# HAHHHD/mllp

Measured on AMD Instinct MI355X. Metric: LP instances/sec (fwd+bwd) on Netlib batch; achieved HBM GB/s on CSR SpMM, higher is better.
Workload: dtype f32; 1 GPU; netlib_full: BASELINE.json configs[2], 97 instances / 1,074,147 nnz per global batch, one block-diagonal batch per GPU, one Adam step per global batch: fwd + BCE + bwd + gradient all-reduce + Adam, fp32; global_batch=97, instances_rank0=97, nnz_rank0=1074147, hip_graph=False, parallelism=dp1

## Files before the change

### mllp_amd/csrc/api.cpp

```cpp
#include <algorithm>

#include "internal.h"

namespace mllp {

static inline int64_t up16(int64_t x) { return (x + 15) & ~int64_t(15); }

ConvWs conv_ws_carve(float* base, int64_t n, int cin, float** end) {
    const int64_t recw = cin == 16 ? REC_W : 8;
    float* p = base;
    auto take = [&](int64_t floats) {
        float* q = p;
        p += up16(floats);
        return q;
    };
    ConvWs w;
    w.derived = take(DERIVED_W);
    w.qp = take(n * cin);
    w.t = take(n);
    w.Z = take(n * cin);
    w.aux = take(n * 4);
    w.rec = take(n * recw);
    w.dqp = take(n * cin);
    w.dsdt = take(n * 2);
// ... 154 lines not shown
    TRY(c1v.pre(s));
    TRY(c1v.dst(s));
    TRY(c1v.stat(s));
    TRY(c1c.pre(a));
    TRY(c1c.dst(a));
    TRY(c1c.stat(a));
#undef REC
#undef WAIT
    TRY(fork_to(a, s, g->ev[0]));
#undef TRY
    return model_finalize(g, P, w, false, grads, s);
}

static bool use_fused(const mllp_graph* g) {
    if (g->path == 1 || !g->fused_built) return false;
    if (g->path == 2) return true;
    return g->nnz < ((int64_t)32 << 20);
}

}

using namespace mllp;

extern "C" int mllp_spmm_csr_f32(const mllp_graph_t* g, int transpose, const float* d_H, float* d_Y, void* stream) {
    REQUIRE(g && d_H && d_Y, "null argument");
    const Orient& o = transpose ? g->At : g->A;
    return launch_spmm(o, d_H, d_Y, o.scratch, (hipStream_t)stream);
}

extern "C" int mllp_spmm_csr_bf16(const mllp_graph_t* g, int transpose, const void* d_H_bf16, float* d_Y, void* stream) {
    REQUIRE(g && d_H_bf16 && d_Y, "null argument");
    const Orient& o = transpose ? g->At : g->A;
    const Tiled& tl = o.tiled[TILED_SPMM];
// ... 2 lines not shown
    if (tl.n_tiles == 0) {
        if (o.n_dst > 0) MLLP_HIP_TRY(hipMemsetAsync(d_Y, 0, (size_t)o.n_dst * 16 * sizeof(float), (hipStream_t)stream));
        return MLLP_OK;
    }
    return launch_spmm_tiled_bf16(tl, o.n_dst, o.n_src, d_H_bf16, d_Y, (hipStream_t)stream);
}

extern "C" int mllp_graph_invalidate_inputs(mllp_graph_t* g) {
    REQUIRE(g, "null graph");
    g->bound_x1 = g->bound_x2 = g->bound_labels = nullptr;
    return MLLP_OK;
}

extern "C" int mllp_graph_set_path(mllp_graph_t* g, int path) {
    REQUIRE(g, "null graph");
    REQUIRE(path >= 0 && path <= 2, "path must be 0 (by size), 1 (generic / LDS-tiled sweeps) or 2 (fused latency-regime kernels)");
    if (path == 2 && !g->fused_built) {
        const int rc = fused_graph_build(g, g->h_csr_ptr.data(), g->h_csc_ptr.data());
        if (rc) return rc;
    }
    g->path = path;
    g->folded_ws = g->folded_params = nullptr;
    return MLLP_OK;
}

extern "C" int mllp_tiled_geometry(int variant, int32_t* rows_per_tile, int32_t* cols_per_block,
                                   int32_t* bundle_capacity) {
    REQUIRE(rows_per_tile && cols_per_block && bundle_capacity, "null argument");
    REQUIRE(variant >= 0 && variant <= 4, "variant must be 0 (SpMM), 1 (attention forward), 2 / 4 (attention backward, source- / destination-major) or 3 (layer-1 sweeps)");
    int a, b, c;
    tiled_geometry(variant, &a, &b, &c);
    *rows_per_tile = a; *cols_per_block = b; *bundle_capacity = c;
// ... 117 lines not shown
                       d_logits, nullptr, w.head_partials, s);
}

extern "C" int mllp_gnn_backward(const mllp_graph_t* g, const float* d_params, const float* d_x1, const float* d_x2,
                                 void* d_ws, const float* d_dlogits, float* d_grads, void* stream) {
    REQUIRE(g && d_params && d_x1 && d_x2 && d_ws && d_dlogits && d_grads, "null argument");
    hipStream_t s = (hipStream_t)stream;
    ModelWs w = model_ws(g, (float*)d_ws);
    int rc;
    REQUIRE(g->ws_ptr == d_ws && g->ws_path == (use_fused(g) ? 1 : 0),
            "no mllp_gnn_forward on this workspace with the current path (mllp_graph_set_path between forward and backward?)");
    if (use_fused(g)) {
        const FusedModel m{d_params, w, d_x1, d_x2, nullptr, 0.0f, nullptr};
        if ((rc = fused_bind(const_cast<mllp_graph*>(g), d_x1, d_x2, nullptr, s))) return rc;
        if ((rc = fused_head_backward(g, m, d_dlogits, s))) return rc;
        return fused_backward(g, m, false, d_grads, nullptr, s);
    }
    if ((rc = launch_head(1, g->N, w.h3v, d_params + OFF_FC, d_params + OFF_FC + FEAT, g->inv_n, nullptr, 0.0f,
                          d_dlogits, nullptr, w.d3v, w.head_partials, s))) return rc;
    if ((rc = fork_to(s, g->aux, g->ev[1]))) return rc;
    if ((rc = launch_head_finalize(w.head_partials, head_blocks_for(g->N), d_grads + OFF_FC, nullptr, g->aux))) return rc;
    return model_backward_body(g, d_params, d_x1, d_x2, w, d_grads, s);
}

static int input_grads_body(const mllp_graph* g, const float* x1, const float* x2, const ModelWs& w, float* dx1,
                            float* dx2, float* dval, hipStream_t s) {
    int rc;
    auto edge = [&](int c, const float* x_src, int accumulate) {
        const bool t = MODEL_CONV[c].dst_is_var;
        return launch_edge_grad(t ? g->At : g->A, g->nnz, MODEL_CONV[c].cin, w.c[c], x_src, t ? g->at_pos : nullptr, dval,
                                accumulate, s);
// ... 5 lines not shown
    if ((rc = edge(CONV_1C, x1, 0)) || (rc = edge(CONV_2C, w.h1v, 1)) || (rc = edge(CONV_1V, x2, 1)) ||
        (rc = edge(CONV_2V, w.h1c, 1))) return rc;
    return edge(CONV_3V, w.h2c, 1);
}

extern "C" int mllp_gnn_loss_step(const mllp_graph_t* g, const float* d_params, const float* d_x1, const float* d_x2,
                                  const float* d_labels, float inv_batch, void* d_ws, float* d_logits, float* d_loss,
                                  float* d_grads, void* stream) {
    REQUIRE(g && d_params && d_x1 && d_x2 && d_labels && d_ws && d_logits && d_loss && d_grads, "null argument");
    hipStream_t s = (hipStream_t)stream;
    ModelWs w = model_ws(g, (float*)d_ws);
    int rc;
    const_cast<mllp_graph*>(g)->folded_ws = const_cast<mllp_graph*>(g)->folded_params = nullptr;
    if (use_fused(g)) {
        const FusedModel m{d_params, w, d_x1, d_x2, d_labels, inv_batch, d_logits};
        if ((rc = fused_forward(const_cast<mllp_graph*>(g), m, 2, s))) return rc;
        return fused_backward(g, m, true, d_grads, d_loss, s);
    }
    if ((rc = model_forward_body(g, d_params, d_x1, d_x2, w, s))) return rc;
    if ((rc = launch_head(2, g->N, w.h3v, d_params + OFF_FC, d_params + OFF_FC + FEAT, g->inv_n, d_labels, inv_batch,
                          nullptr, d_logits, w.d3v, w.head_partials, s))) return rc;
    if ((rc = fork_to(s, g->aux, g->ev[1]))) return rc;
    if ((rc = launch_head_finalize(w.head_partials, head_blocks_for(g->N), d_grads + OFF_FC, d_loss, g->aux))) return rc;
    return model_backward_body(g, d_params, d_x1, d_x2, w, d_grads, s);
}

extern "C" int mllp_gnn_input_grads_scratch_bytes(const mllp_graph_t* g, int64_t* bytes) {
    REQUIRE(g && bytes, "null argument");
    *bytes = up16(MLLP_NUM_PARAMS) * (int64_t)sizeof(float);
    return MLLP_OK;
}

// ... 18 lines not shown
extern "C" int mllp_gnn_train_step(const mllp_graph_t* g, float* d_params, const float* d_x1, const float* d_x2,
                                   const float* d_labels, float inv_batch, void* d_ws, float* d_logits, float* d_loss,
                                   float* d_grads, float* d_exp_avg, float* d_exp_avg_sq, float* d_state, float eps,
                                   int flags, void* stream) {
    REQUIRE(g && d_params && d_x1 && d_x2 && d_labels && d_ws && d_logits && d_loss && d_grads, "null argument");
    REQUIRE(d_exp_avg && d_exp_avg_sq && d_state, "null optimizer state");
    REQUIRE((flags & ~1) == 0, "flags: bit 0 = the folded weights in the workspace are current");
    hipStream_t s = (hipStream_t)stream;
    int rc;
    mllp_graph* gm = const_cast<mllp_graph*>(g);
    if (use_fused(g)) {
        ModelWs w = model_ws(g, (float*)d_ws);
        const FusedModel m{d_params, w, d_x1, d_x2, d_labels, inv_batch, d_logits};
        const bool skip = (flags & 1) != 0 && gm->folded_ws == d_ws && gm->folded_params == d_params;
        gm->folded_ws = gm->folded_params = nullptr;
        if ((rc = fused_forward(gm, m, 2, s, skip))) return rc;
        const FusedAdam a = {d_params, d_exp_avg, d_exp_avg_sq, d_state, eps, (int)MLLP_NUM_PARAMS};
        if ((rc = fused_backward(g, m, true, d_grads, d_loss, s, &a))) return rc;
        gm->folded_ws = d_ws;
        gm->folded_params = d_params;
        return MLLP_OK;
    }
    gm->folded_ws = gm->folded_params = nullptr;
    if ((rc = mllp_gnn_loss_step(g, d_params, d_x1, d_x2, d_labels, inv_batch, d_ws, d_logits, d_loss, d_grads, stream)))
        return rc;
    return launch_adam(d_params, d_grads, d_exp_avg, d_exp_avg_sq, d_state, eps, 1.0f, MLLP_NUM_PARAMS, s);
}

extern "C" int mllp_gnn_small_step_limits(int64_t limits[4]) {
    REQUIRE(limits, "null argument");
    limits[0] = SMALL_STEP_MAX_NODES; limits[1] = SMALL_STEP_MAX_NNZ;
    limits[2] = SMALL_STEP_THREADS; limits[3] = SMALL_STEP_LDS_BYTES;
    return MLLP_OK;
// ... 70 lines not shown
```

### mllp_amd/csrc/fused_kernels.hip

```cpp
#include <algorithm>
#include <vector>

#include "device_utils.h"
#include "host_graph.h"
#include "internal.h"
#include "node_bodies.h"

namespace mllp {

typedef float f32x4m __attribute__((ext_vector_type(4)));

#ifdef MLLP_TIMING_BUILD
static int g_fused_abl = [] {
    const char* e = getenv("MLLP_FUSED_ABL");
    return e ? atoi(e) : 0;
}();
#define FUSED_ABL(bit) ((J.abl & (bit)) != 0)
__device__ unsigned long long g_fused_stamps[8192 * 8];
__device__ unsigned long long g_fused_stamps1[8192 * 8];
#define FUSED_STAMP(k)                                                                      \
    {                                                                                       \
        __builtin_amdgcn_sched_barrier(0);                                                  \
        const unsigned long long now_ = __builtin_amdgcn_s_memtime();                       \
        __builtin_amdgcn_sched_barrier(0);                                                  \
        stamp_sum[k] += now_ - stamp_last;                                                  \
        stamp_last = now_;                                                                  \
    }
#else
#define FUSED_ABL(bit) false
#define FUSED_STAMP(k)
#endif

constexpr int FT = 768;
constexpr int FW = FT / 64;
constexpr int RT = 1024;
constexpr int MAXJOBS = 2;

constexpr int NP = FUSED_NP;
static_assert(NP == FUSED_PARTS, "partition count");

struct PartTiers {
    int row0, n_block, n_wave, n_group, n_base;
};
struct ItemsDev {
    const int* __restrict__ sptr;
// ... 321 lines not shown
        if (J.head == 2) *reinterpret_cast<float4*>(J.g_out + (size_t)p.row * 16 + 4 * part) = p.g;
    }
    p.row = -1;
}

struct FwdNext {
    RowSlot r;
    float4 xd;
    int2 en;
    int lrow;
    SlotReq q;
};
__device__ __forceinline__ void fwd16_row(const FwdJob16& J, const FwdW16& W, const PartTiers& P, const RowSlot& r,
                                          const float4& xd, int2& en, int lrow, const SlotReq& q1, int it2, FwdNext& nx,
                                          FwdPending& pend, int part, int lane, float* merge_lds, float* tiles, HeadAcc& ha
#ifdef MLLP_TIMING_BUILD
                                          , unsigned long long (&stamp_sum)[8], unsigned long long& stamp_last
#endif
) {
    FUSED_STAMP(0)
    const int n_mine = FUSED_ABL(256) ? 0 : slot_count(r);
    Gather4 gt;
    gather4_issue(J.s, J.x_src, r, n_mine, 0, part, en, gt);
    nx.r = slot_make(q1);
    nx.xd = ld4(J.x_dst + (size_t)max(nx.r.row, 0) * 16 + 4 * part);
    nx.en = first_entries_any<4>(J.s, nx.r, part);
    nx.lrow = J.perm[max(nx.r.row, 0)];
    nx.q = item_request<4>(J.s, P, max(it2, 0), lane);
    float4 qp;
    float t;
    {
        float ax_[4];
        tile_put(tiles, xd, lane);
        tile_rows(tiles, lane, ax_);
// ... 95 lines not shown
    ha.b = wave_sum(ha.b);
    ha.l = wave_sum(ha.l);
    if (lane < 4) {
        float* d = head_lds + wave * 18 + 4 * lane;
        d[0] = ha.w.x; d[1] = ha.w.y; d[2] = ha.w.z; d[3] = ha.w.w;
    }
    if (lane == 0) { head_lds[wave * 18 + 16] = ha.b; head_lds[wave * 18 + 17] = ha.l; }
    __syncthreads();
    if (tid < 18) {
        float v = 0.0f;
        for (int w = 0; w < NW; ++w) v += head_lds[w * 18 + tid];
        head_part[(size_t)blockIdx.x * 18 + tid] = v;
    }
}

__global__ __launch_bounds__(FT) void fused_fwd16_kernel(FwdLaunch16 A) {
    __shared__ FwdW16 Ws_[MAXJOBS];
    __shared__ float merge_lds[FW * 20];
    __shared__ float head_lds[FW * 18];
    __shared__ float tiles_[FW * 3 * TILE];
    const int tid = threadIdx.x, lane = tid & 63, wave = tid >> 6, part = lane & 3;
    for (int j = 0; j < A.n_jobs; ++j) {
        const FwdJob16& J = A.job[j];
        FwdW16& W = Ws_[j];
        if (wave == 0) matB_store(W.BPq, matB(J.D + OFF_PQ, 16, lane), lane);
        if (wave == 1) matB_store(W.BWv, matB(J.p.Wv, 16, lane), lane);
        if (wave == 2) matB_store(W.BWs, matB(J.p.Ws, 16, lane), lane);
        if (tid < 16) {
            W.pq0[tid] = J.D[OFF_PQ0 + tid];
            W.Pt[tid] = J.D[OFF_PT + tid];
            W.bv[tid] = J.p.bv[tid];
            W.we[tid] = J.p.we[tid];
            W.bs[tid] = J.p.bs[tid];
            W.fcw[tid] = J.head ? J.fcw[tid] : 0.0f;
        }
        if (tid == 0) {
            W.pt0 = J.D[OFF_PT0];
            W.fcb = J.head ? J.fcb[0] : 0.0f;
        }
    }
    __syncthreads();
    float* tiles = tiles_ + wave * 3 * TILE;
    HeadAcc ha;
    ha.w = f4zero(); ha.b = 0.0f; ha.l = 0.0f;
#ifdef MLLP_TIMING_BUILD
    unsigned long long stamp_sum[8] = {0, 0, 0, 0, 0, 0, 0, 0};
    unsigned long long stamp_last = __builtin_amdgcn_s_memtime();
    const unsigned long long stamp_begin = stamp_last;
#define STAMP_ARGS , stamp_sum, stamp_last
#else
#define STAMP_ARGS
#endif
    const int px = blockIdx.x % NP, bi = blockIdx.x / NP, gp = gridDim.x / NP;
    const int gw = bi * FW + wave;
    float* head_part = nullptr;
    for (int j = 0; j < A.n_jobs; ++j) {
        const FwdJob16& J = A.job[j];
        const PartTiers P = J.s.part[px];
        if (J.head == 2) head_part = J.head_part;
        const RowSlot none = empty_slot();
        FwdPending pend;
        pend.row = -1;
        for (int k = bi; k < P.n_block; k += gp) {
            const RowSlot r = block_slot<4>(J.s, P.row0 + k, tid);
            const float4 xd = ld4(J.x_dst + (size_t)r.row * 16 + 4 * part);
            int2 en = first_entries<4>(J.s, r, part);
            const int lrow = J.head ? J.perm[r.row] : 0;
            FwdNext nx;
            fwd16_row(J, Ws_[j], P, r, xd, en, lrow, empty_request(), -1, nx, pend, part, lane, merge_lds, tiles, ha STAMP_ARGS);
        }
        WaveList wl = wave_list(J.s, px, gw);
        for (int c0 = 0; c0 < wl.L; c0 += 64) {
            wave_list_chunk(wl, c0, lane);
            int it = wave_list_get(wl, 0), it1 = wave_list_get(wl, 1);
            RowSlot r = it >= 0 ? item_slot<4>(J.s, P, it, lane) : none;
            float4 xd = r.row >= 0 ? ld4(J.x_dst + (size_t)r.row * 16 + 4 * part) : f4zero();
            int2 en = first_entries<4>(J.s, r, part);
            int lrow = (J.head && r.row >= 0) ? J.perm[r.row] : 0;
            SlotReq q1 = item_request<4>(J.s, P, max(it1, 0), lane);
            if (it1 < 0) q1.row = -1;
            asm volatile("" : "+v"(xd.x), "+v"(xd.y), "+v"(xd.z), "+v"(xd.w), "+v"(en.x), "+v"(en.y), "+v"(lrow),
                              "+v"(q1.sb), "+v"(q1.se));
            for (int k = 0; it >= 0; ++k) {
                const int it2 = wave_list_get(wl, k + 2);
                FwdNext nx;
                fwd16_row(J, Ws_[j], P, r, xd, en, lrow, q1, it2, nx, pend, part, lane, merge_lds, tiles, ha STAMP_ARGS);
#ifdef MLLP_TIMING_BUILD
                stamp_sum[7] += 1;
#endif
                r = nx.r; xd = nx.xd; en = nx.en; lrow = nx.lrow; q1 = nx.q;
                it = it1; it1 = it2;
            }
        }
        fwd16_flush(J, pend, part);
    }
#ifdef MLLP_TIMING_BUILD
    if (lane == 0 && A.job[0].abl >= 0) {
        stamp_sum[6] = __builtin_amdgcn_s_memtime() - stamp_begin;
        unsigned long long* d = g_fused_stamps + (size_t)(blockIdx.x * FW + wave) * 8;
        for (int k = 0; k < 8; ++k) d[k] = stamp_sum[k];
    }
#endif
    if (head_part) head_partials_store<FW>(ha, head_lds, head_part, tid);
}

struct FwdJob1 {
    ItemsDev s;
    const float* __restrict__ x_dst;
    const float* __restrict__ D;
    ConvParams p;
    float* __restrict__ h;
    float* __restrict__ Z;
// ... 359 lines not shown
        asm volatile("" :: "v"(cg[0]), "v"(cdq[1]), "v"(csc[2]), "v"(cx[3]), "v"(cz[0]), "v"(ce[1]));
        return;
    }
#pragma unroll
    for (int s = 0; s < 4; ++s) {
        acc[0] = __builtin_amdgcn_mfma_f32_16x16x4f32(cg[s], cx[s], acc[0], 0, 0, 0);
        acc[1] = __builtin_amdgcn_mfma_f32_16x16x4f32(cg[s], cz[s], acc[1], 0, 0, 0);
        acc[2] = __builtin_amdgcn_mfma_f32_16x16x4f32(cg[s], ce[s], acc[2], 0, 0, 0);
        acc[3] = __builtin_amdgcn_mfma_f32_16x16x4f32(cdq[s], cx[s], acc[3], 0, 0, 0);
        acc[4] = __builtin_amdgcn_mfma_f32_16x16x4f32(cdq[s], ce[s], acc[4], 0, 0, 0);
        acc[5] = __builtin_amdgcn_mfma_f32_16x16x4f32(csc[s], cx[s], acc[5], 0, 0, 0);
        acc[6] = __builtin_amdgcn_mfma_f32_16x16x4f32(csc[s], ce[s], acc[6], 0, 0, 0);
    }
}

__global__ __launch_bounds__(FT) void fused_bwd16_kernel(BwdLaunch16 A) {
    __shared__ BwdW16 Ws_[MAXJOBS];
    __shared__ float merge_lds[FW * 20];
    __shared__ float tiles_[FW * TB_N * TILE];
    const int tid = threadIdx.x, lane = tid & 63, wave = tid >> 6, part = lane & 3;
    for (int j = 0; j < A.n_jobs; ++j) {
        const BwdJob16& J = A.job[j];
        BwdW16& W = Ws_[j];
        if (wave == 0) matB_store(W.BWvT, matB_t(J.p.Wv, 16, lane), lane);
        if (wave == 1) matB_store(W.BPq, matB(J.D + OFF_PQ, 16, lane), lane);
        if (wave == 2) matB_store(W.BWsT, matB_t(J.p.Ws, 16, lane), lane);
        if (wave == 3) matB_store(W.BPqT, matB_t(J.D + OFF_PQ, 16, lane), lane);
        if (tid < 16) {
            W.pq0[tid] = J.D[OFF_PQ0 + tid];
            W.Pt[tid] = J.D[OFF_PT + tid];
            W.Pb[tid] = J.D[OFF_PB + tid];
            W.bv[tid] = J.p.bv[tid];
            W.we[tid] = J.p.we[tid];
        }
        if (tid == 0) W.pt0 = J.D[OFF_PT0];
    }
    __syncthreads();
    float* tiles = tiles_ + wave * TB_N * TILE;
    const int px = blockIdx.x % NP, bi = blockIdx.x / NP, gp = gridDim.x / NP;
    const int gw = bi * FW + wave;
    for (int j = 0; j < A.n_jobs; ++j) {
        const BwdJob16& J = A.job[j];
        const PartTiers P = J.s.part[px];
        f32x4m acc[STAT_TILES];
#pragma unroll
        for (int i = 0; i < STAT_TILES; ++i) acc[i] = splat4(0.0f);
        const RowSlot none = empty_slot();
        for (int k = bi; k < P.n_block; k += gp) {
            const RowSlot r = block_slot<4>(J.s, P.row0 + k, tid);
            BwdRow rd;
            bwd16_fetch(J, r, part, rd);
            int2 en = first_entries<4>(J.s, r, part);
            RowSlot rn;
            bwd16_row(J, Ws_[j], P, r, rd, en, -1, rn, part, lane, merge_lds, tiles, acc);
        }
        WaveList wl = wave_list(J.s, px, gw);
        for (int c0 = 0; c0 < wl.L; c0 += 64) {
            wave_list_chunk(wl, c0, lane);
            int it = wave_list_get(wl, 0);
            RowSlot r = it >= 0 ? item_slot<4>(J.s, P, it, lane) : none;
            BwdRow rd;
            bwd16_fetch(J, r, part, rd);
            int2 en = first_entries<4>(J.s, r, part);
            for (int k = 0; it >= 0; ++k) {
                const int itn = wave_list_get(wl, k + 1);
                RowSlot rn;
                bwd16_row(J, Ws_[j], P, r, rd, en, itn, rn, part, lane, merge_lds, tiles, acc);
                r = rn;
                it = itn;
            }
        }
        __syncthreads();
        float* red = tiles_;
#pragma unroll
        for (int i = 0; i < STAT_TILES; ++i) {
#pragma unroll
            for (int q = 0; q < 4; ++q) red[wave * 256 + ((lane >> 4) * 4 + q) * 16 + (lane & 15)] = acc[i][q];
            __syncthreads();
            if (tid < 256) {
                float v = 0.0f;
                for (int w = 0; w < FW; ++w) v += red[w * 256 + tid];
                J.stats[(size_t)blockIdx.x * STAT_FLOATS + i * 256 + tid] = v;
            }
            __syncthreads();
        }
    }
}

struct SrcJob16 {
    ItemsDev s;
    const float* __restrict__ x;
    const float* __restrict__ rec;
    float* __restrict__ dx;
    const float* __restrict__ addp;
    float addw;
    int mask;
};
struct SrcLaunch16 {
    SrcJob16 job[MAXJOBS];
    int n_jobs;
};
// ... 630 lines not shown
    J.head = 0;
#ifdef MLLP_TIMING_BUILD
    J.abl = g_fused_abl;
#endif
    return J;
}
static FwdJob1 fwd_job1(const FusedOrient& o, const FusedModel& m, int c, const float* x_dst, float* h) {
    const ConvWs& w = m.w.c[c];
    FwdJob1 J = {};
    J.s = items_dev(o, 1);
    J.x_dst = x_dst; J.D = w.derived; J.p = conv_params_at(conv_at(m.P, c), MODEL_CONV[c].cin);
    J.h = h; J.Z = w.Z; J.aux = w.aux;
    return J;
}

int fused_forward(mllp_graph* g, const FusedModel& m, int head_mode, hipStream_t s, bool skip_prep) {
    const int G = fused_grid(g);
    const ModelWs& w = m.w;
    int rc;
    if ((rc = fused_bind(g, m.x1, m.x2, head_mode == 2 ? m.labels : nullptr, s))) return rc;
    if (!skip_prep && (rc = model_param_prep(m.P, w, s))) return rc;
    {
        FwdLaunch1 L = {};
        L.n_jobs = 2;
        L.job[0] = fwd_job1(g->FAt, m, CONV_1V, g->x1_p, w.h1v);
        L.job[1] = fwd_job1(g->FA, m, CONV_1C, g->x2_p, w.h1c);
        hipLaunchKernelGGL(fused_fwd1_kernel, dim3(G), dim3(FT), 0, s, L);
        if ((rc = check_launch("fused_fwd1"))) return rc;
    }
    {
        FwdLaunch16 L = {};
        L.n_jobs = 2;
        L.job[0] = fwd_job16(g->FAt, m, CONV_2V, w.h1c, w.h1v, w.h2v);
        L.job[1] = fwd_job16(g->FA, m, CONV_2C, w.h1v, w.h1c, w.h2c);
        L.job[0].perm = g->perm_v; L.job[1].perm = g->perm_c;
        hipLaunchKernelGGL(fused_fwd16_kernel, dim3(G), dim3(FT), 0, s, L);
        if ((rc = check_launch("fused_fwd16 layer 2"))) return rc;
    }
    {
        FwdLaunch16 L = {};
        L.n_jobs = 1;
        L.job[0] = fwd_job16(g->FAt, m, CONV_3V, w.h2c, w.h2v, w.h3v);
        FwdJob16& J = L.job[0];
        J.head = head_mode;
        J.fcw = m.P + OFF_FC; J.fcb = m.P + OFF_FC + FEAT; J.inv_n = g->inv_n_p; J.labels = g->labels_p; J.perm = g->perm_v;
        J.inv_batch = m.inv_batch;
        J.logits = m.logits; J.g_out = w.d3v; J.head_part = w.head_partials;
        hipLaunchKernelGGL(fused_fwd16_kernel, dim3(G), dim3(FT), 0, s, L);
        if ((rc = check_launch("fused_fwd16 layer 3"))) return rc;
    }
    return MLLP_OK;
}

int fused_head_backward(const mllp_graph* g, const FusedModel& m, const float* dlogits, hipStream_t s) {
    const int G = fused_grid(g);
    hipLaunchKernelGGL(fused_head_bwd_kernel, dim3(G), dim3(RT), 0, s, (int)g->N, m.w.h3v, m.P + OFF_FC, dlogits, g->perm_v,
                       m.w.d3v, m.w.head_partials);
    return check_launch("fused_head_bwd");
}

static BwdJob16 bwd_job16(const FusedOrient& o, const FusedModel& m, int c, const float* x_src, const float* x_dst,
                          const float* h, const float* dh_a, const float* dh_b, float* dx_dst, bool need_rec, bool mask_dx) {
// ... 15 lines not shown
    SrcJob16 J = {};
    J.s = items_dev(o_src_major, 2);
    J.x = x_rows; J.rec = w.rec; J.dx = dx;
    J.addp = add ? add : x_rows; J.addw = add ? 1.0f : 0.0f; J.mask = 1;
    return J;
}
static BwdJob1 bwd_job1(const FusedOrient& o, const FusedModel& m, int c, const float* x_dst, const float* g_masked) {
    const ConvWs& w = m.w.c[c];
    BwdJob1 J = {};
    J.s = items_dev(o, 1);
    J.x_dst = x_dst; J.D = w.derived; J.p = conv_params_at(conv_at(m.P, c), MODEL_CONV[c].cin);
    J.g = g_masked; J.Z = w.Z; J.aux = w.aux; J.stats = w.stats;
    return J;
}

int fused_backward(const mllp_graph* g, const FusedModel& m, bool premasked, float* grads, float* loss, hipStream_t s,
                   const FusedAdam* adam) {
    const int G = fused_grid(g);
    const ModelWs& w = m.w;
    int rc;
    const FusedOrient& A = g->FA;
    const FusedOrient& At = g->FAt;
    {
        BwdLaunch16 L = {};
        L.n_jobs = 1;
        L.job[0] = bwd_job16(At, m, CONV_3V, w.h2c, w.h2v, premasked ? nullptr : w.h3v, w.d3v, nullptr, w.d2v, true, true);
        hipLaunchKernelGGL(fused_bwd16_kernel, dim3(G), dim3(FT), 0, s, L);
        if ((rc = check_launch("fused_bwd16 C3"))) return rc;
    }
    {
        SrcLaunch16 S = {};
        S.n_jobs = 1;
        S.job[0] = src_job16(A, w.c[CONV_3V], w.h2c, w.d2c, nullptr);
        hipLaunchKernelGGL(fused_src16_kernel, dim3(2 * G), dim3(FT), 0, s, S);
        if ((rc = check_launch("fused_src16 C3"))) return rc;
        BwdLaunch16 L = {};
        L.n_jobs = 1;
        L.job[0] = bwd_job16(At, m, CONV_2V, w.h1c, w.h1v, nullptr, w.d2v, nullptr, w.d1v, true, true);
        hipLaunchKernelGGL(fused_bwd16_kernel, dim3(G), dim3(FT), 0, s, L);
        if ((rc = check_launch("fused_bwd16 C2V"))) return rc;
    }
    {
        BwdLaunch16 L = {};
        L.n_jobs = 1;
        L.job[0] = bwd_job16(A, m, CONV_2C, w.h1v, w.h1c, nullptr, w.d2c, nullptr, w.d1c, true, true);
        hipLaunchKernelGGL(fused_bwd16_kernel, dim3(G), dim3(FT), 0, s, L);
        if ((rc = check_launch("fused_bwd16 C2C"))) return rc;
        SrcLaunch16 S = {};
        S.n_jobs = 2;
        S.job[0] = src_job16(A, w.c[CONV_2V], w.h1c, w.d1c_b, w.d1c);
        S.job[1] = src_job16(At, w.c[CONV_2C], w.h1v, w.d1v_b, w.d1v);
        hipLaunchKernelGGL(fused_src16_kernel, dim3(2 * G), dim3(FT), 0, s, S);
        if ((rc = check_launch("fused_src16 C2V + C2C"))) return rc;
    }
    {
        BwdLaunch1 L = {};
        L.n_jobs = 2;
        L.job[0] = bwd_job1(A, m, CONV_1C, g->x2_p, w.d1c_b);
        L.job[1] = bwd_job1(At, m, CONV_1V, g->x1_p, w.d1v_b);
        hipLaunchKernelGGL(fused_bwd1_kernel, dim3(G), dim3(FT), 0, s, L);
        if ((rc = check_launch("fused_bwd1"))) return rc;
    }
// ... 37 lines not shown
```

### mllp_amd/csrc/internal.h

```cpp
#pragma once
#include <hip/hip_runtime.h>
#include <stdint.h>

#include <algorithm>
#include <string>
#include <vector>

#include "../../include/mllp_hip.h"

namespace mllp {

constexpr int FEAT = 16;
constexpr int BLOCK = 256;
constexpr int REC_W = 40;
constexpr int STAT_TILES = 7;
constexpr int STAT_FLOATS = STAT_TILES * 256;
constexpr int STAT_BLOCKS_MAX = 256;

void set_error(const std::string& msg);
int fail(int code, const std::string& msg);
int hip_fail(hipError_t e, const char* what);

#define MLLP_HIP_TRY(expr)                                              \
    do {                                                                \
// ... 308 lines not shown
                       unsigned char* mask, int* index, float* stats, hipStream_t s);

struct FusedModel {
    const float* P;
    const ModelWs& w;
    const float *x1, *x2, *labels;
    float inv_batch;
    float* logits;
};
int model_param_prep(const float* P, const ModelWs& w, hipStream_t s);
int model_finalize(const mllp_graph* g, const float* P, const ModelWs& w, bool reduced, float* grads, hipStream_t s);
int fused_graph_build(mllp_graph* g, const int* h_csr_ptr, const int* h_csc_ptr);
int fused_grid(const mllp_graph* g);
int fused_refill_values(mllp_graph* g, hipStream_t s);
int fused_bind(mllp_graph* g, const float* x1, const float* x2, const float* labels, hipStream_t s);
int fused_forward(mllp_graph* g, const FusedModel& m, int head_mode, hipStream_t s, bool skip_prep = false);
int fused_head_backward(const mllp_graph* g, const FusedModel& m, const float* dlogits, hipStream_t s);
struct FusedAdam {
    float *params, *m, *v, *state;
    float eps;
    int n;
};
int fused_backward(const mllp_graph* g, const FusedModel& m, bool premasked, float* grads, float* loss, hipStream_t s,
                   const FusedAdam* adam = nullptr);

}
```

Before: 292,000 instances/s.

## Chain layer-3 forward with C3 backward and co-launch the C2V/C2C backward sweeps

```diff
diff --git a/mllp_amd/csrc/api.cpp b/mllp_amd/csrc/api.cpp
--- a/mllp_amd/csrc/api.cpp
+++ b/mllp_amd/csrc/api.cpp
@@ -192,9 +192,10 @@
 
 static bool use_fused(const mllp_graph* g) {
     if (g->path == 1 || !g->fused_built) return false;
-    if (g->path == 2) return true;
+    if (g->path == 2 || g->path == 3) return true;
     return g->nnz < ((int64_t)32 << 20);
 }
+static int fused_schedule(const mllp_graph* g) { return g->path == 3 ? FUSED_SEPARATE : FUSED_CHAINED; }
 
 }
 
@@ -227,8 +228,9 @@
 
 extern "C" int mllp_graph_set_path(mllp_graph_t* g, int path) {
     REQUIRE(g, "null graph");
-    REQUIRE(path >= 0 && path <= 2, "path must be 0 (by size), 1 (generic / LDS-tiled sweeps) or 2 (fused latency-regime kernels)");
-    if (path == 2 && !g->fused_built) {
+    REQUIRE(path >= 0 && path <= 3, "path must be 0 (by size), 1 (generic / LDS-tiled sweeps), 2 (fused latency-regime kernels) "
+                                    "or 3 (the fused kernels with one launch per sweep)");
+    if ((path == 2 || path == 3) && !g->fused_built) {
         const int rc = fused_graph_build(g, g->h_csr_ptr.data(), g->h_csc_ptr.data());
         if (rc) return rc;
     }
@@ -376,7 +378,7 @@
         const FusedModel m{d_params, w, d_x1, d_x2, nullptr, 0.0f, nullptr};
         if ((rc = fused_bind(const_cast<mllp_graph*>(g), d_x1, d_x2, nullptr, s))) return rc;
         if ((rc = fused_head_backward(g, m, d_dlogits, s))) return rc;
-        return fused_backward(g, m, false, d_grads, nullptr, s);
+        return fused_backward(g, m, false, d_grads, nullptr, s, nullptr, fused_schedule(g));
     }
     if ((rc = launch_head(1, g->N, w.h3v, d_params + OFF_FC, d_params + OFF_FC + FEAT, g->inv_n, nullptr, 0.0f,
                           d_dlogits, nullptr, w.d3v, w.head_partials, s))) return rc;
@@ -412,8 +414,9 @@
     const_cast<mllp_graph*>(g)->folded_ws = const_cast<mllp_graph*>(g)->folded_params = nullptr;
     if (use_fused(g)) {
         const FusedModel m{d_params, w, d_x1, d_x2, d_labels, inv_batch, d_logits};
-        if ((rc = fused_forward(const_cast<mllp_graph*>(g), m, 2, s))) return rc;
-        return fused_backward(g, m, true, d_grads, d_loss, s);
+        const int sched = fused_schedule(g);
+        if ((rc = fused_forward(const_cast<mllp_graph*>(g), m, 2, s, false, sched == FUSED_CHAINED))) return rc;
+        return fused_backward(g, m, true, d_grads, d_loss, s, nullptr, sched);
     }
     if ((rc = model_forward_body(g, d_params, d_x1, d_x2, w, s))) return rc;
     if ((rc = launch_head(2, g->N, w.h3v, d_params + OFF_FC, d_params + OFF_FC + FEAT, g->inv_n, d_labels, inv_batch,
@@ -462,9 +465,10 @@
         const FusedModel m{d_params, w, d_x1, d_x2, d_labels, inv_batch, d_logits};
         const bool skip = (flags & 1) != 0 && gm->folded_ws == d_ws && gm->folded_params == d_params;
         gm->folded_ws = gm->folded_params = nullptr;
-        if ((rc = fused_forward(gm, m, 2, s, skip))) return rc;
+        const int sched = fused_schedule(g);
+        if ((rc = fused_forward(gm, m, 2, s, skip, sched == FUSED_CHAINED))) return rc;
         const FusedAdam a = {d_params, d_exp_avg, d_exp_avg_sq, d_state, eps, (int)MLLP_NUM_PARAMS};
-        if ((rc = fused_backward(g, m, true, d_grads, d_loss, s, &a))) return rc;
+        if ((rc = fused_backward(g, m, true, d_grads, d_loss, s, &a, sched))) return rc;
         gm->folded_ws = d_ws;
         gm->folded_params = d_params;
         return MLLP_OK;
diff --git a/mllp_amd/csrc/fused_kernels.hip b/mllp_amd/csrc/fused_kernels.hip
--- a/mllp_amd/csrc/fused_kernels.hip
+++ b/mllp_amd/csrc/fused_kernels.hip
@@ -26,9 +26,13 @@
         stamp_sum[k] += now_ - stamp_last;                                                  \
         stamp_last = now_;                                                                  \
     }
+#define STAMP_PARAMS , unsigned long long (&stamp_sum)[8], unsigned long long& stamp_last
+#define STAMP_ARGS , stamp_sum, stamp_last
 #else
 #define FUSED_ABL(bit) false
 #define FUSED_STAMP(k)
+#define STAMP_PARAMS
+#define STAMP_ARGS
 #endif
 
 constexpr int FT = 768;
@@ -380,10 +384,7 @@
 __device__ __forceinline__ void fwd16_row(const FwdJob16& J, const FwdW16& W, const PartTiers& P, const RowSlot& r,
                                           const float4& xd, int2& en, int lrow, const SlotReq& q1, int it2, FwdNext& nx,
                                           FwdPending& pend, int part, int lane, float* merge_lds, float* tiles, HeadAcc& ha
-#ifdef MLLP_TIMING_BUILD
-                                          , unsigned long long (&stamp_sum)[8], unsigned long long& stamp_last
-#endif
-) {
+                                          STAMP_PARAMS) {
     FUSED_STAMP(0)
     const int n_mine = FUSED_ABL(256) ? 0 : slot_count(r);
     Gather4 gt;
@@ -509,31 +510,75 @@
     }
 }
 
+__device__ __forceinline__ void fwd16_weights(const FwdJob16& J, FwdW16& W, int tid) {
+    const int lane = tid & 63, wave = tid >> 6;
+    if (wave == 0) matB_store(W.BPq, matB(J.D + OFF_PQ, 16, lane), lane);
+    if (wave == 1) matB_store(W.BWv, matB(J.p.Wv, 16, lane), lane);
+    if (wave == 2) matB_store(W.BWs, matB(J.p.Ws, 16, lane), lane);
+    if (tid < 16) {
+        W.pq0[tid] = J.D[OFF_PQ0 + tid];
+        W.Pt[tid] = J.D[OFF_PT + tid];
+        W.bv[tid] = J.p.bv[tid];
+        W.we[tid] = J.p.we[tid];
+        W.bs[tid] = J.p.bs[tid];
+        W.fcw[tid] = J.head ? J.fcw[tid] : 0.0f;
+    }
+    if (tid == 0) {
+        W.pt0 = J.D[OFF_PT0];
+        W.fcb = J.head ? J.fcb[0] : 0.0f;
+    }
+}
+
+__device__ __forceinline__ void fwd16_job(const FwdJob16& J, const FwdW16& W, float* merge_lds, float* tiles, HeadAcc& ha,
+                                          int tid STAMP_PARAMS) {
+    const int lane = tid & 63, wave = tid >> 6, part = lane & 3;
+    const int px = blockIdx.x % NP, bi = blockIdx.x / NP, gp = gridDim.x / NP;
+    const int gw = bi * FW + wave;
+    const PartTiers P = J.s.part[px];
+    const RowSlot none = empty_slot();
+    FwdPending pend;
+    pend.row = -1;
+    for (int k = bi; k < P.n_block; k += gp) {
+        const RowSlot r = block_slot<4>(J.s, P.row0 + k, tid);
+        const float4 xd = ld4(J.x_dst + (size_t)r.row * 16 + 4 * part);
+        int2 en = first_entries<4>(J.s, r, part);
+        const int lrow = J.head ? J.perm[r.row] : 0;
+        FwdNext nx;
+        fwd16_row(J, W, P, r, xd, en, lrow, empty_request(), -1, nx, pend, part, lane, merge_lds, tiles, ha STAMP_ARGS);
+    }
+    WaveList wl = wave_list(J.s, px, gw);
+    for (int c0 = 0; c0 < wl.L; c0 += 64) {
+        wave_list_chunk(wl, c0, lane);
+        int it = wave_list_get(wl, 0), it1 = wave_list_get(wl, 1);
+        RowSlot r = it >= 0 ? item_slot<4>(J.s, P, it, lane) : none;
+        float4 xd = r.row >= 0 ? ld4(J.x_dst + (size_t)r.row * 16 + 4 * part) : f4zero();
+        int2 en = first_entries<4>(J.s, r, part);
+        int lrow = (J.head && r.row >= 0) ? J.perm[r.row] : 0;
+        SlotReq q1 = item_request<4>(J.s, P, max(it1, 0), lane);
+        if (it1 < 0) q1.row = -1;
+        asm volatile("" : "+v"(xd.x), "+v"(xd.y), "+v"(xd.z), "+v"(xd.w), "+v"(en.x), "+v"(en.y), "+v"(lrow),
+                          "+v"(q1.sb), "+v"(q1.se));
+        for (int k = 0; it >= 0; ++k) {
+            const int it2 = wave_list_get(wl, k + 2);
+            FwdNext nx;
+            fwd16_row(J, W, P, r, xd, en, lrow, q1, it2, nx, pend, part, lane, merge_lds, tiles, ha STAMP_ARGS);
+#ifdef MLLP_TIMING_BUILD
+            stamp_sum[7] += 1;
+#endif
+            r = nx.r; xd = nx.xd; en = nx.en; lrow = nx.lrow; q1 = nx.q;
+            it = it1; it1 = it2;
+        }
+    }
+    fwd16_flush(J, pend, part);
+}
+
 __global__ __launch_bounds__(FT) void fused_fwd16_kernel(FwdLaunch16 A) {
     __shared__ FwdW16 Ws_[MAXJOBS];
     __shared__ float merge_lds[FW * 20];
     __shared__ float head_lds[FW * 18];
     __shared__ float tiles_[FW * 3 * TILE];
-    const int tid = threadIdx.x, lane = tid & 63, wave = tid >> 6, part = lane & 3;
-    for (int j = 0; j < A.n_jobs; ++j) {
-        const FwdJob16& J = A.job[j];
-        FwdW16& W = Ws_[j];
-        if (wave == 0) matB_store(W.BPq, matB(J.D + OFF_PQ, 16, lane), lane);
-        if (wave == 1) matB_store(W.BWv, matB(J.p.Wv, 16, lane), lane);
-        if (wave == 2) matB_store(W.BWs, matB(J.p.Ws, 16, lane), lane);
-        if (tid < 16) {
-            W.pq0[tid] = J.D[OFF_PQ0 + tid];
-            W.Pt[tid] = J.D[OFF_PT + tid];
-            W.bv[tid] = J.p.bv[tid];
-            W.we[tid] = J.p.we[tid];
-            W.bs[tid] = J.p.bs[tid];
-            W.fcw[tid] = J.head ? J.fcw[tid] : 0.0f;
-        }
-        if (tid == 0) {
-            W.pt0 = J.D[OFF_PT0];
-            W.fcb = J.head ? J.fcb[0] : 0.0f;
-        }
-    }
+    const int tid = threadIdx.x, wave = tid >> 6;
+    for (int j = 0; j < A.n_jobs; ++j) fwd16_weights(A.job[j], Ws_[j], tid);
     __syncthreads();
     float* tiles = tiles_ + wave * 3 * TILE;
     HeadAcc ha;
@@ -542,55 +587,15 @@
     unsigned long long stamp_sum[8] = {0, 0, 0, 0, 0, 0, 0, 0};
     unsigned long long stamp_last = __builtin_amdgcn_s_memtime();
     const unsigned long long stamp_begin = stamp_last;
-#define STAMP_ARGS , stamp_sum, stamp_last
-#else
-#define STAMP_ARGS
 #endif
-    const int px = blockIdx.x % NP, bi = blockIdx.x / NP, gp = gridDim.x / NP;
-    const int gw = bi * FW + wave;
     float* head_part = nullptr;
     for (int j = 0; j < A.n_jobs; ++j) {
         const FwdJob16& J = A.job[j];
-        const PartTiers P = J.s.part[px];
         if (J.head == 2) head_part = J.head_part;
-        const RowSlot none = empty_slot();
-        FwdPending pend;
-        pend.row = -1;
-        for (int k = bi; k < P.n_block; k += gp) {
-            const RowSlot r = block_slot<4>(J.s, P.row0 + k, tid);
-            const float4 xd = ld4(J.x_dst + (size_t)r.row * 16 + 4 * part);
-            int2 en = first_entries<4>(J.s, r, part);
-            const int lrow = J.head ? J.perm[r.row] : 0;
-            FwdNext nx;
-            fwd16_row(J, Ws_[j], P, r, xd, en, lrow, empty_request(), -1, nx, pend, part, lane, merge_lds, tiles, ha STAMP_ARGS);
-        }
-        WaveList wl = wave_list(J.s, px, gw);
-        for (int c0 = 0; c0 < wl.L; c0 += 64) {
-            wave_list_chunk(wl, c0, lane);
-            int it = wave_list_get(wl, 0), it1 = wave_list_get(wl, 1);
-            RowSlot r = it >= 0 ? item_slot<4>(J.s, P, it, lane) : none;
-            float4 xd = r.row >= 0 ? ld4(J.x_dst + (size_t)r.row * 16 + 4 * part) : f4zero();
-            int2 en = first_entries<4>(J.s, r, part);
-            int lrow = (J.head && r.row >= 0) ? J.perm[r.row] : 0;
-            SlotReq q1 = item_request<4>(J.s, P, max(it1, 0), lane);
-            if (it1 < 0) q1.row = -1;
-            asm volatile("" : "+v"(xd.x), "+v"(xd.y), "+v"(xd.z), "+v"(xd.w), "+v"(en.x), "+v"(en.y), "+v"(lrow),
-                              "+v"(q1.sb), "+v"(q1.se));
-            for (int k = 0; it >= 0; ++k) {
-                const int it2 = wave_list_get(wl, k + 2);
-                FwdNext nx;
-                fwd16_row(J, Ws_[j], P, r, xd, en, lrow, q1, it2, nx, pend, part, lane, merge_lds, tiles, ha STAMP_ARGS);
+        fwd16_job(J, Ws_[j], merge_lds, tiles, ha, tid STAMP_ARGS);
+    }
 #ifdef MLLP_TIMING_BUILD
-                stamp_sum[7] += 1;
-#endif
-                r = nx.r; xd = nx.xd; en = nx.en; lrow = nx.lrow; q1 = nx.q;
-                it = it1; it1 = it2;
-            }
-        }
-        fwd16_flush(J, pend, part);
-    }
-#ifdef MLLP_TIMING_BUILD
-    if (lane == 0 && A.job[0].abl >= 0) {
+    if ((tid & 63) == 0 && A.job[0].abl >= 0) {
         stamp_sum[6] = __builtin_amdgcn_s_memtime() - stamp_begin;
         unsigned long long* d = g_fused_stamps + (size_t)(blockIdx.x * FW + wave) * 8;
         for (int k = 0; k < 8; ++k) d[k] = stamp_sum[k];
@@ -980,77 +985,109 @@
     }
 }
 
+__device__ __forceinline__ void bwd16_weights(const BwdJob16& J, BwdW16& W, int tid) {
+    const int lane = tid & 63, wave = tid >> 6;
+    if (wave == 0) matB_store(W.BWvT, matB_t(J.p.Wv, 16, lane), lane);
+    if (wave == 1) matB_store(W.BPq, matB(J.D + OFF_PQ, 16, lane), lane);
+    if (wave == 2) matB_store(W.BWsT, matB_t(J.p.Ws, 16, lane), lane);
+    if (wave == 3) matB_store(W.BPqT, matB_t(J.D + OFF_PQ, 16, lane), lane);
+    if (tid < 16) {
+        W.pq0[tid] = J.D[OFF_PQ0 + tid];
+        W.Pt[tid] = J.D[OFF_PT + tid];
+        W.Pb[tid] = J.D[OFF_PB + tid];
+        W.bv[tid] = J.p.bv[tid];
+        W.we[tid] = J.p.we[tid];
+    }
+    if (tid == 0) W.pt0 = J.D[OFF_PT0];
+}
+
+__device__ __forceinline__ void bwd16_job(const BwdJob16& J, const BwdW16& W, float* merge_lds, float* tiles_, int tid) {
+    const int lane = tid & 63, wave = tid >> 6, part = lane & 3;
+    float* tiles = tiles_ + wave * TB_N * TILE;
+    const int px = blockIdx.x % NP, bi = blockIdx.x / NP, gp = gridDim.x / NP;
+    const int gw = bi * FW + wave;
+    const PartTiers P = J.s.part[px];
+    f32x4m acc[STAT_TILES];
+#pragma unroll
+    for (int i = 0; i < STAT_TILES; ++i) acc[i] = splat4(0.0f);
+    const RowSlot none = empty_slot();
+    for (int k = bi; k < P.n_block; k += gp) {
+        const RowSlot r = block_slot<4>(J.s, P.row0 + k, tid);
+        BwdRow rd;
+        bwd16_fetch(J, r, part, rd);
+        int2 en = first_entries<4>(J.s, r, part);
+        RowSlot rn;
+        bwd16_row(J, W, P, r, rd, en, -1, rn, part, lane, merge_lds, tiles, acc);
+    }
+    WaveList wl = wave_list(J.s, px, gw);
+    for (int c0 = 0; c0 < wl.L; c0 += 64) {
+        wave_list_chunk(wl, c0, lane);
+        int it = wave_list_get(wl, 0);
+        RowSlot r = it >= 0 ? item_slot<4>(J.s, P, it, lane) : none;
+        BwdRow rd;
+        bwd16_fetch(J, r, part, rd);
+        int2 en = first_entries<4>(J.s, r, part);
+        for (int k = 0; it >= 0; ++k) {
+            const int itn = wave_list_get(wl, k + 1);
+            RowSlot rn;
+            bwd16_row(J, W, P, r, rd, en, itn, rn, part, lane, merge_lds, tiles, acc);
+            r = rn;
+            it = itn;
+        }
+    }
+    __syncthreads();
+    float* red = tiles_;
+#pragma unroll
+    for (int i = 0; i < STAT_TILES; ++i) {
+#pragma unroll
+        for (int q = 0; q < 4; ++q) red[wave * 256 + ((lane >> 4) * 4 + q) * 16 + (lane & 15)] = acc[i][q];
+        __syncthreads();
+        if (tid < 256) {
+            float v = 0.0f;
+            for (int w = 0; w < FW; ++w) v += red[w * 256 + tid];
+            J.stats[(size_t)blockIdx.x * STAT_FLOATS + i * 256 + tid] = v;
+        }
+        __syncthreads();
+    }
+}
+
 __global__ __launch_bounds__(FT) void fused_bwd16_kernel(BwdLaunch16 A) {
     __shared__ BwdW16 Ws_[MAXJOBS];
     __shared__ float merge_lds[FW * 20];
     __shared__ float tiles_[FW * TB_N * TILE];
-    const int tid = threadIdx.x, lane = tid & 63, wave = tid >> 6, part = lane & 3;
-    for (int j = 0; j < A.n_jobs; ++j) {
-        const BwdJob16& J = A.job[j];
-        BwdW16& W = Ws_[j];
-        if (wave == 0) matB_store(W.BWvT, matB_t(J.p.Wv, 16, lane), lane);
-        if (wave == 1) matB_store(W.BPq, matB(J.D + OFF_PQ, 16, lane), lane);
-        if (wave == 2) matB_store(W.BWsT, matB_t(J.p.Ws, 16, lane), lane);
-        if (wave == 3) matB_store(W.BPqT, matB_t(J.D + OFF_PQ, 16, lane), lane);
-        if (tid < 16) {
-            W.pq0[tid] = J.D[OFF_PQ0 + tid];
-            W.Pt[tid] = J.D[OFF_PT + tid];
-            W.Pb[tid] = J.D[OFF_PB + tid];
-            W.bv[tid] = J.p.bv[tid];
-            W.we[tid] = J.p.we[tid];
-        }
-        if (tid == 0) W.pt0 = J.D[OFF_PT0];
-    }
+    const int tid = threadIdx.x;
+    for (int j = 0; j < A.n_jobs; ++j) bwd16_weights(A.job[j], Ws_[j], tid);
     __syncthreads();
-    float* tiles = tiles_ + wave * TB_N * TILE;
-    const int px = blockIdx.x % NP, bi = blockIdx.x / NP, gp = gridDim.x / NP;
-    const int gw = bi * FW + wave;
-    for (int j = 0; j < A.n_jobs; ++j) {
-        const BwdJob16& J = A.job[j];
-        const PartTiers P = J.s.part[px];
-        f32x4m acc[STAT_TILES];
-#pragma unroll
-        for (int i = 0; i < STAT_TILES; ++i) acc[i] = splat4(0.0f);
-        const RowSlot none = empty_slot();
-        for (int k = bi; k < P.n_block; k += gp) {
-            const RowSlot r = block_slot<4>(J.s, P.row0 + k, tid);
-            BwdRow rd;
-            bwd16_fetch(J, r, part, rd);
-            int2 en = first_entries<4>(J.s, r, part);
-            RowSlot rn;
-            bwd16_row(J, Ws_[j], P, r, rd, en, -1, rn, part, lane, merge_lds, tiles, acc);
-        }
-        WaveList wl = wave_list(J.s, px, gw);
-        for (int c0 = 0; c0 < wl.L; c0 += 64) {
-            wave_list_chunk(wl, c0, lane);
-            int it = wave_list_get(wl, 0);
-            RowSlot r = it >= 0 ? item_slot<4>(J.s, P, it, lane) : none;
-            BwdRow rd;
-            bwd16_fetch(J, r, part, rd);
-            int2 en = first_entries<4>(J.s, r, part);
-            for (int k = 0; it >= 0; ++k) {
-                const int itn = wave_list_get(wl, k + 1);
-                RowSlot rn;
-                bwd16_row(J, Ws_[j], P, r, rd, en, itn, rn, part, lane, merge_lds, tiles, acc);
-                r = rn;
-                it = itn;
-            }
-        }
-        __syncthreads();
-        float* red = tiles_;
-#pragma unroll
-        for (int i = 0; i < STAT_TILES; ++i) {
-#pragma unroll
-            for (int q = 0; q < 4; ++q) red[wave * 256 + ((lane >> 4) * 4 + q) * 16 + (lane & 15)] = acc[i][q];
-            __syncthreads();
-            if (tid < 256) {
-                float v = 0.0f;
-                for (int w = 0; w < FW; ++w) v += red[w * 256 + tid];
-                J.stats[(size_t)blockIdx.x * STAT_FLOATS + i * 256 + tid] = v;
-            }
-            __syncthreads();
-        }
-    }
+    for (int j = 0; j < A.n_jobs; ++j) bwd16_job(A.job[j], Ws_[j], merge_lds, tiles_, tid);
+}
+
+struct ChainLaunch16 {
+    FwdJob16 fwd;
+    BwdJob16 bwd[MAXJOBS];
+    int n_bwd;
+};
+__global__ __launch_bounds__(FT) void fused_chain16_kernel(ChainLaunch16 A) {
+    __shared__ FwdW16 Wf;
+    __shared__ BwdW16 Wb[MAXJOBS];
+    __shared__ float merge_lds[FW * 20];
+    __shared__ float head_lds[FW * 18];
+    __shared__ float tiles_[FW * TB_N * TILE];
+    const int tid = threadIdx.x, wave = tid >> 6;
+    fwd16_weights(A.fwd, Wf, tid);
+    for (int j = 0; j < A.n_bwd; ++j) bwd16_weights(A.bwd[j], Wb[j], tid);
+    __syncthreads();
+    {
+        HeadAcc ha;
+        ha.w = f4zero(); ha.b = 0.0f; ha.l = 0.0f;
+#ifdef MLLP_TIMING_BUILD
+        unsigned long long stamp_sum[8] = {0, 0, 0, 0, 0, 0, 0, 0};
+        unsigned long long stamp_last = 0;
+#endif
+        fwd16_job(A.fwd, Wf, merge_lds, tiles_ + wave * TB_N * TILE, ha, tid STAMP_ARGS);
+        head_partials_store<FW>(ha, head_lds, A.fwd.head_part, tid);
+    }
+    __syncthreads();
+    for (int j = 0; j < A.n_bwd; ++j) bwd16_job(A.bwd[j], Wb[j], merge_lds, tiles_, tid);
 }
 
 struct SrcJob16 {
@@ -1711,7 +1748,17 @@
     return J;
 }
 
-int fused_forward(mllp_graph* g, const FusedModel& m, int head_mode, hipStream_t s, bool skip_prep) {
+static FwdJob16 fwd_job16_head(const mllp_graph* g, const FusedModel& m, int head_mode) {
+    const ModelWs& w = m.w;
+    FwdJob16 J = fwd_job16(g->FAt, m, CONV_3V, w.h2c, w.h2v, w.h3v);
+    J.head = head_mode;
+    J.fcw = m.P + OFF_FC; J.fcb = m.P + OFF_FC + FEAT; J.inv_n = g->inv_n_p; J.labels = g->labels_p; J.perm = g->perm_v;
+    J.inv_batch = m.inv_batch;
+    J.logits = m.logits; J.g_out = w.d3v; J.head_part = w.head_partials;
+    return J;
+}
+
+int fused_forward(mllp_graph* g, const FusedModel& m, int head_mode, hipStream_t s, bool skip_prep, bool defer_layer3) {
     const int G = fused_grid(g);
     const ModelWs& w = m.w;
     int rc;
@@ -1734,15 +1781,10 @@
         hipLaunchKernelGGL(fused_fwd16_kernel, dim3(G), dim3(FT), 0, s, L);
         if ((rc = check_launch("fused_fwd16 layer 2"))) return rc;
     }
-    {
+    if (!(defer_layer3 && head_mode == 2)) {
         FwdLaunch16 L = {};
         L.n_jobs = 1;
-        L.job[0] = fwd_job16(g->FAt, m, CONV_3V, w.h2c, w.h2v, w.h3v);
-        FwdJob16& J = L.job[0];
-        J.head = head_mode;
-        J.fcw = m.P + OFF_FC; J.fcb = m.P + OFF_FC + FEAT; J.inv_n = g->inv_n_p; J.labels = g->labels_p; J.perm = g->perm_v;
-        J.inv_batch = m.inv_batch;
-        J.logits = m.logits; J.g_out = w.d3v; J.head_part = w.head_partials;
+        L.job[0] = fwd_job16_head(g, m, head_mode);
         hipLaunchKernelGGL(fused_fwd16_kernel, dim3(G), dim3(FT), 0, s, L);
         if ((rc = check_launch("fused_fwd16 layer 3"))) return rc;
     }
@@ -1788,38 +1830,54 @@
     return J;
 }
 
+#ifndef MLLP_FUSED_CHAIN_C2V
+#define MLLP_FUSED_CHAIN_C2V 0
+#endif
+constexpr bool FUSED_CHAIN_C2V = MLLP_FUSED_CHAIN_C2V != 0;
+
 int fused_backward(const mllp_graph* g, const FusedModel& m, bool premasked, float* grads, float* loss, hipStream_t s,
-                   const FusedAdam* adam) {
+                   const FusedAdam* adam, int schedule) {
     const int G = fused_grid(g);
     const ModelWs& w = m.w;
     int rc;
     const FusedOrient& A = g->FA;
     const FusedOrient& At = g->FAt;
-    {
+    const bool chained = schedule == FUSED_CHAINED;
+    const BwdJob16 k1 = bwd_job16(At, m, CONV_3V, w.h2c, w.h2v, premasked ? nullptr : w.h3v, w.d3v, nullptr, w.d2v, true, true);
+    const BwdJob16 k2v = bwd_job16(At, m, CONV_2V, w.h1c, w.h1v, nullptr, w.d2v, nullptr, w.d1v, true, true);
+    const BwdJob16 k3 = bwd_job16(A, m, CONV_2C, w.h1v, w.h1c, nullptr, w.d2c, nullptr, w.d1c, true, true);
+    auto bwd16 = [&](const BwdJob16& a, const BwdJob16* b, const char* what) {
         BwdLaunch16 L = {};
-        L.n_jobs = 1;
-        L.job[0] = bwd_job16(At, m, CONV_3V, w.h2c, w.h2v, premasked ? nullptr : w.h3v, w.d3v, nullptr, w.d2v, true, true);
+        L.n_jobs = b ? 2 : 1;
+        L.job[0] = a;
+        if (b) L.job[1] = *b;
         hipLaunchKernelGGL(fused_bwd16_kernel, dim3(G), dim3(FT), 0, s, L);
-        if ((rc = check_launch("fused_bwd16 C3"))) return rc;
-    }
+        return check_launch(what);
+    };
+    const bool k2v_with_k1 = chained && FUSED_CHAIN_C2V, k2v_with_k3 = chained && !FUSED_CHAIN_C2V;
+    if (chained && premasked) {
+        ChainLaunch16 L = {};
+        L.fwd = fwd_job16_head(g, m, 2);
+        L.bwd[0] = k1;
+        L.n_bwd = 1;
+        if (k2v_with_k1) L.bwd[L.n_bwd++] = k2v;
+        hipLaunchKernelGGL(fused_chain16_kernel, dim3(G), dim3(FT), 0, s, L);
+        if ((rc = check_launch("fused_chain16"))) return rc;
+    } else if ((rc = bwd16(k1, k2v_with_k1 ? &k2v : nullptr, "fused_bwd16 C3"))) return rc;
     {
         SrcLaunch16 S = {};
         S.n_jobs = 1;
         S.job[0] = src_job16(A, w.c[CONV_3V], w.h2c, w.d2c, nullptr);
         hipLaunchKernelGGL(fused_src16_kernel, dim3(2 * G), dim3(FT), 0, s, S);
         if ((rc = check_launch("fused_src16 C3"))) return rc;
-        BwdLaunch16 L = {};
-        L.n_jobs = 1;
-        L.job[0] = bwd_job16(At, m, CONV_2V, w.h1c, w.h1v, nullptr, w.d2v, nullptr, w.d1v, true, true);
-        hipLaunchKernelGGL(fused_bwd16_kernel, dim3(G), dim3(FT), 0, s, L);
-        if ((rc = check_launch("fused_bwd16 C2V"))) return rc;
+    }
+    if (k2v_with_k3) {
+        if ((rc = bwd16(k2v, &k3, "fused_bwd16 C2V + C2C"))) return rc;
+    } else {
+        if (!k2v_with_k1 && (rc = bwd16(k2v, nullptr, "fused_bwd16 C2V"))) return rc;
+        if ((rc = bwd16(k3, nullptr, "fused_bwd16 C2C"))) return rc;
     }
     {
-        BwdLaunch16 L = {};
-        L.n_jobs = 1;
-        L.job[0] = bwd_job16(A, m, CONV_2C, w.h1v, w.h1c, nullptr, w.d2c, nullptr, w.d1c, true, true);
-        hipLaunchKernelGGL(fused_bwd16_kernel, dim3(G), dim3(FT), 0, s, L);
-        if ((rc = check_launch("fused_bwd16 C2C"))) return rc;
         SrcLaunch16 S = {};
         S.n_jobs = 2;
         S.job[0] = src_job16(A, w.c[CONV_2V], w.h1c, w.d1c_b, w.d1c);
diff --git a/mllp_amd/csrc/internal.h b/mllp_amd/csrc/internal.h
--- a/mllp_amd/csrc/internal.h
+++ b/mllp_amd/csrc/internal.h
@@ -346,14 +346,16 @@
 int fused_grid(const mllp_graph* g);
 int fused_refill_values(mllp_graph* g, hipStream_t s);
 int fused_bind(mllp_graph* g, const float* x1, const float* x2, const float* labels, hipStream_t s);
-int fused_forward(mllp_graph* g, const FusedModel& m, int head_mode, hipStream_t s, bool skip_prep = false);
+int fused_forward(mllp_graph* g, const FusedModel& m, int head_mode, hipStream_t s, bool skip_prep = false,
+                  bool defer_layer3 = false);
 int fused_head_backward(const mllp_graph* g, const FusedModel& m, const float* dlogits, hipStream_t s);
 struct FusedAdam {
     float *params, *m, *v, *state;
     float eps;
     int n;
 };
+enum { FUSED_SEPARATE = 0, FUSED_CHAINED = 1 };
 int fused_backward(const mllp_graph* g, const FusedModel& m, bool premasked, float* grads, float* loss, hipStream_t s,
-                   const FusedAdam* adam = nullptr);
-
-}
+                   const FusedAdam* adam = nullptr, int schedule = FUSED_SEPARATE);
+
+}
```

Result: no change. 294,700 instances/s (median of 6 runs) (+0.9%).
